# ElementsProject/lightning

Measured on NVIDIA H100. Metric: secp256k1 verifies/sec, higher is better.
Workload: dtype u32 (8x32-bit limbs, IMAD.WIDE.U32 carry chains)

## Files before the change

include/cln_sigverify.h:

```cpp
#ifndef CLN_SIGVERIFY_H
#define CLN_SIGVERIFY_H

#include <stddef.h>
#include <stdint.h>

#ifdef __cplusplus
extern "C" {
#endif

typedef struct sv_ctx sv_ctx;

#define SV_KIND_ECDSA33 0
#define SV_KIND_ECDSA_XY 1
#define SV_KIND_SCHNORR 2

typedef enum {
    SV_OK = 0,
    SV_ERR_NO_DEVICE = -1,
    SV_ERR_CUDA = -2,
    SV_ERR_NOMEM = -3,
    SV_ERR_ARG = -4,
    SV_ERR_IO = -5
} sv_status;

// ... 156 lines not shown
    uint64_t input_amount, output_amount;
    uint32_t prevouts_off, prevouts_len;
    uint32_t sequences_off, sequences_len;
} sv_tx;
int sv_verify_tx_host(sv_ctx *ctx, int kind, const sv_tx *txs, const uint8_t *scripts, size_t scripts_len,
                      const uint8_t *key, const uint8_t *sig64, size_t n, uint8_t *verdicts, uint8_t *sighash32_out);

int sv_grind_tx_fee_host(sv_ctx *ctx, int kind, const sv_tx *tx, const uint8_t *scripts, size_t scripts_len,
                         const uint8_t *key, const uint8_t *sig64, uint64_t weight, uint32_t min_feerate,
                         uint32_t max_feerate, int64_t *feerate_out, uint64_t *fee_out);

int sv_verify_bolt12_host(sv_ctx *ctx, const char *messagename, const char *fieldname, const uint8_t *blob,
                          size_t blob_len, const uint64_t *off, const uint32_t *len, const uint8_t *xonly32,
                          const uint8_t *sig64, size_t n, int *status, uint8_t *sighash32_out);
int sv_verify_bolt12_tagged_host(sv_ctx *ctx, size_t ntags, const char *const *messagenames, const char *const *fieldnames,
                                 const uint32_t *tag_of, const uint8_t *blob, size_t blob_len, const uint64_t *off,
                                 const uint32_t *len, const uint8_t *xonly32, const uint8_t *sig64, size_t n,
                                 int *status, uint8_t *sighash32_out);

int sv_verify_bolt11_host(sv_ctx *ctx, const uint8_t *blob, size_t blob_len, const uint64_t *off, const uint32_t *len,
                          size_t n, int *status, uint8_t *node_id33_out, uint8_t *hash32_out);

int sv_verify_device(sv_ctx *ctx, int kind, const void *d_msg32, const void *d_key, const void *d_sig64, size_t n,
                     void *d_verdicts, void *d_bitmap, void *stream);
int sv_sync(sv_ctx *ctx, void *stream);
void *sv_get_stream(const sv_ctx *ctx);

long sv_enqueue(sv_ctx *ctx, int kind, const uint8_t msg32[32], const uint8_t *key, const uint8_t sig64[64]);
size_t sv_pending(const sv_ctx *ctx);
int sv_flush(sv_ctx *ctx, uint8_t *verdicts, size_t capacity);

int sv_sha256d_host(sv_ctx *ctx, const uint8_t *data, size_t data_len, const uint64_t *off, const uint32_t *len,
                    size_t n, uint8_t *out32);
int sv_pubkey_parse_host(sv_ctx *ctx, const uint8_t *key33, size_t n, uint8_t *xy64, uint8_t *ok);

enum {
    SV_ST_FE_MUL = 0,
    SV_ST_FE_SQR = 1,
    SV_ST_FE_ADD = 2,
    SV_ST_FE_SUB = 3,
    SV_ST_FE_NEG = 4,
    SV_ST_FE_NORMALIZE = 5,
    SV_ST_FE_INV = 6,
    SV_ST_FE_SQRT = 7,
    SV_ST_FE_MUL3 = 8,
    SV_ST_FE_MUL8 = 9,
    SV_ST_FE_MUL_SMALL = 10,
    SV_ST_FE_DBL = 11,
    SV_ST_FE_B32 = 12,
    SV_ST_U256_MUL_WIDE = 13,
    SV_ST_U256_SQR_WIDE = 14,
    SV_ST_FE_REDUCE512 = 15,
    SV_ST_U256_ADD = 16,
    SV_ST_U256_SUB = 17,
    SV_ST_SC_MUL = 20,
    SV_ST_SC_SQR = 21,
    SV_ST_SC_ADD = 22,
    SV_ST_SC_NEGATE = 23,
    SV_ST_SC_INVERSE = 24,
    SV_ST_SC_REDUCE512 = 25,
    SV_ST_SC_SPLIT_LAMBDA = 26,
    SV_ST_SC_SET_B32 = 27,
    SV_ST_ECMULT_GEN = 28,
    SV_ST_PREPARE_U2 = 29,
    SV_ST_PREPARE_U1 = 30,
    SV_ST_SC_INVERSE_VAR = 31,
    SV_ST_FE_INV_VAR = 32
};
int sv_selftest_host(sv_ctx *ctx, int op, const uint32_t *a, const uint32_t *b, size_t n, uint32_t *out);

#define SV_STG_IN_WORDS 64
#define SV_STG_OUT_WORDS 200
enum {
    SV_STG_GEJ_DOUBLE = 0,
    SV_STG_GEJ_ADD_GE = 1,
    SV_STG_GEJ_ADD_GEJ = 2,
    SV_STG_GE_SET_XO = 3,
    SV_STG_QTABLE_BUILD = 4,
    SV_STG_ECMULT_LADDER_Q = 5,
    SV_STG_ECMULT_HALF_LADDER = 6,
    SV_STG_ECMULT_COMB_ADD = 7,
    SV_STG_SMALL_COMB = 8,
    SV_STG_ECMULT_LADDER = 9,
    SV_STG_NS_LINEAR_FORM = 10
};
int sv_selftest_group_host(sv_ctx *ctx, int op, const uint32_t *in, size_t n, uint32_t *out);

int sv_synth_device(sv_ctx *ctx, int kind, uint64_t seed, size_t n, void *d_msg32, void *d_key, void *d_sig64,
                    void *stream);

typedef struct {
    int device;
    int sm_count;
    int main_block;
    int main_grid;
    int main_regs;
    size_t gtable_bytes;
    size_t scratch_bytes;
    unsigned long long launches;
    size_t l2_persist_bytes;
    size_t l2_max_persist_bytes;
} sv_info;
int sv_get_info(const sv_ctx *ctx, sv_info *info);

int sv_set_profiling(sv_ctx *ctx, int on);
int sv_get_last_timing(sv_ctx *ctx, float *prep_ms, float *main_ms);
int sv_get_last_bolt12_timing(sv_ctx *ctx, float *merkle_ms, float *verify_ms);
int sv_get_last_bolt11_timing(sv_ctx *ctx, float *parse_ms, float *curve_ms);

int sv_probe_imad_peak(sv_ctx *ctx, double *imad_per_sec);
int sv_probe(sv_ctx *ctx, int mode, double *ops_per_sec);

void *sv_host_alloc(size_t bytes);
void sv_host_free(void *p);

#ifdef __cplusplus
}
#endif
#endif
```

lightning_b200/csrc/engine.cu:

```cuda
#include <cuda_runtime.h>
#include <cub/device/device_radix_sort.cuh>
#include <cub/device/device_scan.cuh>
#include <stdio.h>
#include <chrono>
#include <memory>
#include <stdlib.h>
#include <string.h>
#include <string>
#include <vector>

#include "../../include/cln_sigverify.h"
#include "verify.cuh"
#include "bolt12.cuh"
#include "bolt11.cuh"
#include "gossip_store.cuh"
#include "gossip_salvage.cuh"
#include "gossip_funding.cuh"
#include "selftest.cuh"
#include "batch.cuh"

#if !defined(SV_NO_SYNC_INLINE) && !defined(SV_FE_INLINE)
#error "compile with -DSV_FE_INLINE -DSV_MAIN_SYNC (default build) or -DSV_NO_SYNC_INLINE; see lightning_b200/build.py"
#endif
#ifdef SV_MAIN_SYNC
// ... 2980 lines not shown
    if (groups_total) *groups_total = groups;
    if (groups_failed) *groups_failed = failed;
    if (!idx.empty()) {
        size_t c = idx.size();
        CK(cudaMemcpyAsync(d_idx, idx.data(), 4 * c, cudaMemcpyHostToDevice, st));
        u8* g_msg = reinterpret_cast<u8*>(d_pts);
        u8* g_key = g_msg + 32 * c;
        u8* g_sig = g_key + 32 * c;
        u8* g_v = g_sig + 64 * c;
        k_sb_gather<<<(unsigned)((c + 255) / 256), 256, 0, st>>>(d_idx, c, ctx->d_msg, ctx->d_key, ctx->d_sig, g_msg, g_key, g_sig);
        ctx->launches += 1;
        rc = launch_verify(ctx, SV_KIND_SCHNORR, g_msg, g_key, g_sig, c, g_v, nullptr, st);
        if (rc) return rc;
        k_mixed_scatter<<<(unsigned)((c + 255) / 256), 256, 0, st>>>(d_idx, c, g_v, d_out);
        ctx->launches += 1;
        CK(cudaGetLastError());
    }
    CK(cudaMemcpyAsync(verdicts, d_out, n, cudaMemcpyDeviceToHost, st));
    CK(cudaStreamSynchronize(st));
    return SV_OK;
}

extern "C" long sv_enqueue(sv_ctx* ctx, int kind, const uint8_t msg32[32], const uint8_t* key, const uint8_t sig64[64]) {
    size_t ks = sv_key_size(kind);
    if (!ctx || ks == 0 || !msg32 || !key || !sig64) return SV_ERR_ARG;
    sv_queue_item it;
    it.kind = kind;
    memcpy(it.msg, msg32, 32);
    memset(it.key, 0, 64);
    memcpy(it.key, key, ks);
    memcpy(it.sig, sig64, 64);
    ctx->queue.push_back(it);
    return (long)ctx->queue.size() - 1;
}
extern "C" size_t sv_pending(const sv_ctx* ctx) { return ctx ? ctx->queue.size() : 0; }

extern "C" int sv_flush(sv_ctx* ctx, uint8_t* verdicts, size_t capacity) {
    if (!ctx || (!verdicts && !ctx->queue.empty())) return SV_ERR_ARG;
    size_t total = ctx->queue.size();
    if (capacity < total) return SV_ERR_ARG;
    for (int kind = 0; kind < 3; kind++) {
        size_t ks = sv_key_size(kind);
        std::vector<size_t> idx;
        for (size_t i = 0; i < total; i++)
            if (ctx->queue[i].kind == kind) idx.push_back(i);
        if (idx.empty()) continue;
        size_t m = idx.size();
        std::vector<u8> msg(32 * m), key(ks * m), sig(64 * m), out(m);
        for (size_t j = 0; j < m; j++) {
            const sv_queue_item& it = ctx->queue[idx[j]];
            memcpy(&msg[32 * j], it.msg, 32);
            memcpy(&key[ks * j], it.key, ks);
            memcpy(&sig[64 * j], it.sig, 64);
        }
        int rc = sv_verify_host(ctx, kind, msg.data(), key.data(), sig.data(), m, out.data());
        if (rc) return rc;
        for (size_t j = 0; j < m; j++) verdicts[idx[j]] = out[j];
    }
    ctx->queue.clear();
    return SV_OK;
}

extern "C" int sv_selftest_host(sv_ctx* ctx, int op, const uint32_t* a, const uint32_t* b, size_t n, uint32_t* out) {
    if (!ctx || op < 0 || op > SV_ST_FE_INV_VAR || (n && (!a || !b || !out))) return SV_ERR_ARG;
    if (n == 0) return SV_OK;
    dev_guard dg__;
    CK(dg__.enter(ctx->device));
    dev_buf<u32> ta, tb, to;
    int rc = ta.reserve(ctx, n * 32, n * 32);
    if (!rc) rc = tb.reserve(ctx, n * 32, n * 32);
    if (!rc) rc = to.reserve(ctx, n * 64, n * 64);
    if (rc) return rc;
    cudaStream_t st = ctx->stream;
    CK(cudaMemcpyAsync(ta, a, n * 32, cudaMemcpyHostToDevice, st));
    CK(cudaMemcpyAsync(tb, b, n * 32, cudaMemcpyHostToDevice, st));
    k_selftest<<<(unsigned)((n + 127) / 128), 128, 0, st>>>(op, ta, tb, n, to, ctx->d_gtab);
    ctx->launches += 1;
    CK(cudaGetLastError());
    CK(cudaMemcpyAsync(out, to, n * 64, cudaMemcpyDeviceToHost, st));
    CK(cudaStreamSynchronize(st));
    return SV_OK;
}
extern "C" int sv_selftest_group_host(sv_ctx* ctx, int op, const uint32_t* in, size_t n, uint32_t* out) {
    if (!ctx || op < 0 || op > SV_STG_NS_LINEAR_FORM || (n && (!in || !out))) return SV_ERR_ARG;
    if (n == 0) return SV_OK;
    dev_guard dg__;
    CK(dg__.enter(ctx->device));
    const size_t ib = n * 4 * SV_STG_IN_WORDS, ob = n * 4 * SV_STG_OUT_WORDS;
    dev_buf<u32> ti, to;
    int rc = ti.reserve(ctx, ib, ib);
    if (!rc) rc = to.reserve(ctx, ob, ob);
    if (rc) return rc;
    cudaStream_t st = ctx->stream;
    CK(cudaMemcpyAsync(ti, in, ib, cudaMemcpyHostToDevice, st));
    k_selftest_group<<<(unsigned)((n + 127) / 128), 128, 0, st>>>(op, ti, n, to, ctx->d_gtab);
    ctx->launches += 1;
    CK(cudaGetLastError());
    CK(cudaMemcpyAsync(out, to, ob, cudaMemcpyDeviceToHost, st));
    CK(cudaStreamSynchronize(st));
    return SV_OK;
}

extern "C" int sv_synth_device(sv_ctx* ctx, int kind, uint64_t seed, size_t n, void* d_msg32, void* d_key,
                               void* d_sig64, void* stream) {
    if (!ctx || sv_key_size(kind) == 0 || (n && (!d_msg32 || !d_key || !d_sig64))) return SV_ERR_ARG;
    if (n == 0) return SV_OK;
    dev_guard dg__;
    CK(dg__.enter(ctx->device));
    cudaStream_t st = stream ? (cudaStream_t)stream : ctx->stream;
    unsigned grid = (unsigned)((n + 127) / 128);
    if (kind == SV_KIND_ECDSA33)
        k_synth<SV_KIND_ECDSA33><<<grid, 128, 0, st>>>(seed, n, ctx->d_gtab, (u8*)d_msg32, (u8*)d_key, (u8*)d_sig64);
    else if (kind == SV_KIND_ECDSA_XY)
        k_synth<SV_KIND_ECDSA_XY><<<grid, 128, 0, st>>>(seed, n, ctx->d_gtab, (u8*)d_msg32, (u8*)d_key, (u8*)d_sig64);
    else
        k_synth<SV_KIND_SCHNORR><<<grid, 128, 0, st>>>(seed, n, ctx->d_gtab, (u8*)d_msg32, (u8*)d_key, (u8*)d_sig64);
    ctx->launches += 1;
    CK(cudaGetLastError());
    return SV_OK;
}

extern "C" int sv_probe(sv_ctx* ctx, int mode, double* ops_per_sec) {
    if (!ctx || !ops_per_sec || mode < 0 || mode > 10) return SV_ERR_ARG;
    dev_guard dg__;
    CK(dg__.enter(ctx->device));
    const int iters = (mode == 2 || mode == 3 || mode >= 9) ? 2000 : 4000;
    const int blocks = mode >= 9 ? 1 : ctx->sm_count * 8, threads = mode >= 9 ? 32 : 256;
    using event_ptr = std::unique_ptr<CUevent_st, cudaError_t (*)(cudaEvent_t)>;
    cudaEvent_t e0 = nullptr, e1 = nullptr;
    CK(cudaEventCreate(&e0));
    event_ptr own0(e0, cudaEventDestroy);
    CK(cudaEventCreate(&e1));
    event_ptr own1(e1, cudaEventDestroy);
    float best = 1e30f;
    for (int rep = 0; rep < 4; rep++) {
        CK(cudaEventRecord(e0, ctx->stream));
        switch (mode) {
            case 0: k_probe_imad_wide<<<blocks, threads, 0, ctx->stream>>>(iters, ctx->d_sink); break;
            case 1: k_probe_cmad4<<<blocks, threads, 0, ctx->stream>>>(iters, ctx->d_sink); break;
            case 2: k_probe_fe<0><<<blocks, threads, 0, ctx->stream>>>(iters, ctx->d_sink); break;
            case 3: k_probe_fe<1><<<blocks, threads, 0, ctx->stream>>>(iters, ctx->d_sink); break;
            case 4: k_probe_chain8<<<blocks, threads, 0, ctx->stream>>>(iters, ctx->d_sink); break;
            case 5: k_probe_carry_save<<<blocks, threads, 0, ctx->stream>>>(iters, ctx->d_sink); break;
            case 6: k_probe_imad32<<<blocks, threads, 0, ctx->stream>>>(iters, ctx->d_sink); break;
            case 8: k_probe_dfma<<<blocks, threads, 0, ctx->stream>>>(iters, ctx->d_sink); break;
            case 9: k_probe_fe<0><<<blocks, threads, 0, ctx->stream>>>(iters, ctx->d_sink); break;
            case 10: k_probe_fe<1><<<blocks, threads, 0, ctx->stream>>>(iters, ctx->d_sink); break;
            default: k_probe_addc<<<blocks, threads, 0, ctx->stream>>>(iters, ctx->d_sink); break;
        }
        CK(cudaEventRecord(e1, ctx->stream));
        CK(cudaEventSynchronize(e1));
        float ms = 0;
        CK(cudaEventElapsedTime(&ms, e0, e1));
        if (rep > 0 && ms < best) best = ms;
        ctx->launches += 1;
    }
    static const double per_iter[11] = {32.0, 32.0, 2.0, 2.0, 32.0, 32.0, 32.0, 64.0, 32.0, 2.0, 1.0};
    *ops_per_sec = per_iter[mode] * iters * (mode >= 9 ? 1.0 : (double)blocks * threads) / (best * 1e-3);
    return SV_OK;
}
extern "C" int sv_probe_imad_peak(sv_ctx* ctx, double* imad_per_sec) { return sv_probe(ctx, 0, imad_per_sec); }

extern "C" void* sv_host_alloc(size_t bytes) {
    void* p = nullptr;
    if (cudaHostAlloc(&p, bytes ? bytes : 1, cudaHostAllocDefault) != cudaSuccess) return nullptr;
    return p;
}
// ... 4 lines not shown
```

lightning_b200/csrc/fe.cuh:

```cuda
#pragma once
#include "u256.cuh"

struct fe {
    u32 v[8];
};

#define SV_P0 0xFFFFFC2Fu
#define SV_P1 0xFFFFFFFEu
#define SV_PC 977u

SV_HD void fe_set_zero(fe& r) {
    SV_UNROLL
    for (int i = 0; i < 8; i++) r.v[i] = 0;
}
SV_HD void fe_set_u32(fe& r, u32 x) {
    fe_set_zero(r);
    r.v[0] = x;
}

SV_HD bool fe_gte_p(const fe& a) {
    u32 hi = a.v[7] & a.v[6] & a.v[5] & a.v[4] & a.v[3] & a.v[2];
    return (hi == 0xFFFFFFFFu) && ((a.v[1] == 0xFFFFFFFFu) || (a.v[1] == SV_P1 && a.v[0] >= SV_P0));
}

// ... 31 lines not shown
    asm("mad.lo.cc.u32 %0, %3, 977, %0;\n\t"
        "addc.cc.u32 %1, %1, %3;\n\t"
        "addc.u32 %2, 0, 0;"
        : "+r"(r.v[0]), "+r"(r.v[1]), "=r"(k)
        : "r"(c));
    if (k) {
        u32 c2;
        asm("add.cc.u32 %0, %0, 1;\n\t"
            "addc.cc.u32 %1, %1, 0;\n\t"
            "addc.cc.u32 %2, %2, 0;\n\t"
            "addc.cc.u32 %3, %3, 0;\n\t"
            "addc.cc.u32 %4, %4, 0;\n\t"
            "addc.cc.u32 %5, %5, 0;\n\t"
            "addc.u32 %6, 0, 0;"
            : "+r"(r.v[2]), "+r"(r.v[3]), "+r"(r.v[4]), "+r"(r.v[5]), "+r"(r.v[6]), "+r"(r.v[7]), "=r"(c2));
        asm("mad.lo.cc.u32 %0, %2, 977, %0;\n\t"
            "addc.u32 %1, %1, %2;"
            : "+r"(r.v[0]), "+r"(r.v[1])
            : "r"(c2));
    }
#else
    u64 t = (u64)r.v[0] + (u64)c * SV_PC;
    r.v[0] = (u32)t;
    t = (u64)r.v[1] + c + (t >> 32);
    r.v[1] = (u32)t;
    for (int i = 2; i < 8; i++) { t = (u64)r.v[i] + (t >> 32); r.v[i] = (u32)t; }
    u32 c2 = (u32)(t >> 32);
    t = (u64)r.v[0] + (u64)c2 * SV_PC;
    r.v[0] = (u32)t;
    r.v[1] = (u32)((u64)r.v[1] + c2 + (t >> 32));
#endif
}

SV_HD void fe_sub(fe& r, const fe& a, const fe& b) {
    u32 bw = u256_sub(r.v, a.v, b.v);
#if SV_DEVICE_CODE
    u32 k;
    u32 kc = bw * SV_PC;
    asm("sub.cc.u32 %0, %0, %4;\n\t"
        "subc.cc.u32 %1, %1, %3;\n\t"
        "subc.u32 %2, 0, 0;"
        : "+r"(r.v[0]), "+r"(r.v[1]), "=r"(k)
        : "r"(bw), "r"(kc));
    if (k) {
        u32 b2;
        asm("sub.cc.u32 %0, %0, 1;\n\t"
            "subc.cc.u32 %1, %1, 0;\n\t"
            "subc.cc.u32 %2, %2, 0;\n\t"
            "subc.cc.u32 %3, %3, 0;\n\t"
            "subc.cc.u32 %4, %4, 0;\n\t"
            "subc.cc.u32 %5, %5, 0;\n\t"
            "subc.u32 %6, 0, 0;"
            : "+r"(r.v[2]), "+r"(r.v[3]), "+r"(r.v[4]), "+r"(r.v[5]), "+r"(r.v[6]), "+r"(r.v[7]), "=r"(b2));
        b2 &= 1u;
        u32 k2 = b2 * SV_PC;
        asm("sub.cc.u32 %0, %0, %3;\n\t"
            "subc.u32 %1, %1, %2;"
            : "+r"(r.v[0]), "+r"(r.v[1])
            : "r"(b2), "r"(k2));
    }
#else
    u64 d = (u64)r.v[0] - (u64)bw * SV_PC;
    r.v[0] = (u32)d;
    u64 br = (d >> 32) & 1;
    d = (u64)r.v[1] - bw - br;
    r.v[1] = (u32)d;
    br = (d >> 32) & 1;
    for (int i = 2; i < 8; i++) { d = (u64)r.v[i] - br; r.v[i] = (u32)d; br = (d >> 32) & 1; }
    u32 b2 = (u32)br;
    d = (u64)r.v[0] - (u64)b2 * SV_PC;
    r.v[0] = (u32)d;
    br = (d >> 32) & 1;
    r.v[1] = (u32)((u64)r.v[1] - b2 - br);
#endif
}

SV_HD void fe_neg(fe& r, const fe& a) {
    fe z;
    fe_set_zero(z);
    fe_sub(r, z, a);
}
SV_HD void fe_dbl(fe& r, const fe& a) { fe_add(r, a, a); }

SV_HD void fe_reduce512(fe& r, const u32 t[16]) {
#if SV_DEVICE_CODE
    u32 s[10];
    s[0] = t[0];
    asm("add.cc.u32 %0, %9, %17;\n\t"
        "addc.cc.u32 %1, %10, %18;\n\t"
        "addc.cc.u32 %2, %11, %19;\n\t"
        "addc.cc.u32 %3, %12, %20;\n\t"
        "addc.cc.u32 %4, %13, %21;\n\t"
        "addc.cc.u32 %5, %14, %22;\n\t"
        "addc.cc.u32 %6, %15, %23;\n\t"
        "addc.cc.u32 %7, %16, 0;\n\t"
        "addc.u32 %8, 0, 0;"
        : "=r"(s[1]), "=r"(s[2]), "=r"(s[3]), "=r"(s[4]), "=r"(s[5]), "=r"(s[6]), "=r"(s[7]), "=r"(s[8]), "=r"(s[9])
        : "r"(t[8]), "r"(t[9]), "r"(t[10]), "r"(t[11]), "r"(t[12]), "r"(t[13]), "r"(t[14]), "r"(t[15]),
          "r"(t[1]), "r"(t[2]), "r"(t[3]), "r"(t[4]), "r"(t[5]), "r"(t[6]), "r"(t[7]));
#ifdef SV_REDUCE_NOACC
    u32 pe[8];
    asm("mul.lo.u32 %0, %8, %12;\n\t"
        "mul.hi.u32 %1, %8, %12;\n\t"
        "mul.lo.u32 %2, %9, %12;\n\t"
        "mul.hi.u32 %3, %9, %12;\n\t"
        "mul.lo.u32 %4, %10, %12;\n\t"
        "mul.hi.u32 %5, %10, %12;\n\t"
        "mul.lo.u32 %6, %11, %12;\n\t"
        "mul.hi.u32 %7, %11, %12;"
        : "=r"(pe[0]), "=r"(pe[1]), "=r"(pe[2]), "=r"(pe[3]), "=r"(pe[4]), "=r"(pe[5]), "=r"(pe[6]), "=r"(pe[7])
        : "r"(t[8]), "r"(t[10]), "r"(t[12]), "r"(t[14]), "r"(SV_PC));
    asm("add.cc.u32 %0, %0, %10;\n\t"
        "addc.cc.u32 %1, %1, %11;\n\t"
        "addc.cc.u32 %2, %2, %12;\n\t"
        "addc.cc.u32 %3, %3, %13;\n\t"
        "addc.cc.u32 %4, %4, %14;\n\t"
        "addc.cc.u32 %5, %5, %15;\n\t"
        "addc.cc.u32 %6, %6, %16;\n\t"
        "addc.cc.u32 %7, %7, %17;\n\t"
        "addc.cc.u32 %8, %8, 0;\n\t"
        "addc.u32 %9, %9, 0;"
        : "+r"(s[0]), "+r"(s[1]), "+r"(s[2]), "+r"(s[3]), "+r"(s[4]), "+r"(s[5]), "+r"(s[6]), "+r"(s[7]),
          "+r"(s[8]), "+r"(s[9])
        : "r"(pe[0]), "r"(pe[1]), "r"(pe[2]), "r"(pe[3]), "r"(pe[4]), "r"(pe[5]), "r"(pe[6]), "r"(pe[7]));
#else
    asm("mad.lo.cc.u32 %0, %10, %14, %0;\n\t"
        "madc.hi.cc.u32 %1, %10, %14, %1;\n\t"
        "madc.lo.cc.u32 %2, %11, %14, %2;\n\t"
        "madc.hi.cc.u32 %3, %11, %14, %3;\n\t"
        "madc.lo.cc.u32 %4, %12, %14, %4;\n\t"
        "madc.hi.cc.u32 %5, %12, %14, %5;\n\t"
        "madc.lo.cc.u32 %6, %13, %14, %6;\n\t"
        "madc.hi.cc.u32 %7, %13, %14, %7;\n\t"
        "addc.cc.u32 %8, %8, 0;\n\t"
        "addc.u32 %9, %9, 0;"
        : "+r"(s[0]), "+r"(s[1]), "+r"(s[2]), "+r"(s[3]), "+r"(s[4]), "+r"(s[5]), "+r"(s[6]), "+r"(s[7]),
          "+r"(s[8]), "+r"(s[9])
        : "r"(t[8]), "r"(t[10]), "r"(t[12]), "r"(t[14]), "r"(SV_PC));
#endif
    u32 o[8];
    asm("mul.lo.u32 %0, %8, %12;\n\t"
        "mul.hi.u32 %1, %8, %12;\n\t"
        "mul.lo.u32 %2, %9, %12;\n\t"
        "mul.hi.u32 %3, %9, %12;\n\t"
        "mul.lo.u32 %4, %10, %12;\n\t"
        "mul.hi.u32 %5, %10, %12;\n\t"
        "mul.lo.u32 %6, %11, %12;\n\t"
        "mul.hi.u32 %7, %11, %12;"
        : "=r"(o[0]), "=r"(o[1]), "=r"(o[2]), "=r"(o[3]), "=r"(o[4]), "=r"(o[5]), "=r"(o[6]), "=r"(o[7])
        : "r"(t[9]), "r"(t[11]), "r"(t[13]), "r"(t[15]), "r"(SV_PC));
    asm("add.cc.u32 %0, %0, %9;\n\t"
        "addc.cc.u32 %1, %1, %10;\n\t"
        "addc.cc.u32 %2, %2, %11;\n\t"
        "addc.cc.u32 %3, %3, %12;\n\t"
        "addc.cc.u32 %4, %4, %13;\n\t"
        "addc.cc.u32 %5, %5, %14;\n\t"
        "addc.cc.u32 %6, %6, %15;\n\t"
        "addc.cc.u32 %7, %7, %16;\n\t"
        "addc.u32 %8, %8, 0;"
        : "+r"(s[1]), "+r"(s[2]), "+r"(s[3]), "+r"(s[4]), "+r"(s[5]), "+r"(s[6]), "+r"(s[7]), "+r"(s[8]), "+r"(s[9])
        : "r"(o[0]), "r"(o[1]), "r"(o[2]), "r"(o[3]), "r"(o[4]), "r"(o[5]), "r"(o[6]), "r"(o[7]));
    u64 T = ((u64)s[9] << 32) | s[8];
    u64 m = T * SV_PC;
    u64 mid = (m >> 32) + T;
    u32 f0 = (u32)m, f1 = (u32)mid, f2 = (u32)(mid >> 32);
    u32 c;
    asm("add.cc.u32 %0, %9, %17;\n\t"
        "addc.cc.u32 %1, %10, %18;\n\t"
        "addc.cc.u32 %2, %11, %19;\n\t"
        "addc.cc.u32 %3, %12, 0;\n\t"
        "addc.cc.u32 %4, %13, 0;\n\t"
        "addc.cc.u32 %5, %14, 0;\n\t"
        "addc.cc.u32 %6, %15, 0;\n\t"
        "addc.cc.u32 %7, %16, 0;\n\t"
        "addc.u32 %8, 0, 0;"
        : "=r"(r.v[0]), "=r"(r.v[1]), "=r"(r.v[2]), "=r"(r.v[3]), "=r"(r.v[4]), "=r"(r.v[5]), "=r"(r.v[6]),
          "=r"(r.v[7]), "=r"(c)
        : "r"(s[0]), "r"(s[1]), "r"(s[2]), "r"(s[3]), "r"(s[4]), "r"(s[5]), "r"(s[6]), "r"(s[7]), "r"(f0), "r"(f1),
          "r"(f2));
    asm("mad.lo.cc.u32 %0, %3, 977, %0;\n\t"
        "addc.cc.u32 %1, %1, %3;\n\t"
        "addc.u32 %2, %2, 0;"
        : "+r"(r.v[0]), "+r"(r.v[1]), "+r"(r.v[2])
        : "r"(c));
#else
    u64 acc = 0;
    u32 s[10];
    for (int i = 0; i < 8; i++) {
        acc += (u64)t[i] + (u64)t[8 + i] * SV_PC;
        if (i > 0) acc += t[8 + i - 1];
        s[i] = (u32)acc;
        acc >>= 32;
    }
    acc += t[15];
    s[8] = (u32)acc;
    s[9] = (u32)(acc >> 32);
    u64 T = ((u64)s[9] << 32) | s[8];
    u64 m = T * SV_PC;
    u64 mid = (m >> 32) + T;
    u32 f[3] = {(u32)m, (u32)mid, (u32)(mid >> 32)};
    u64 c = 0;
    for (int i = 0; i < 8; i++) {
        c += (u64)s[i] + (i < 3 ? f[i] : 0);
        r.v[i] = (u32)c;
        c >>= 32;
    }
    u32 cc = (u32)c;
    u64 q = (u64)r.v[0] + (u64)cc * SV_PC;
    r.v[0] = (u32)q;
    q = (u64)r.v[1] + cc + (q >> 32);
    r.v[1] = (u32)q;
    r.v[2] = (u32)((u64)r.v[2] + (q >> 32));
#endif
}

#if SV_DEVICE_CODE && !defined(SV_FE_INLINE)
static __device__ __noinline__ fe fe_mul_fn(fe a, fe b) {
    u32 t[16];
    fe r;
    u256_mul_wide(t, a.v, b.v);
    fe_reduce512(r, t);
    return r;
}
static __device__ __noinline__ fe fe_sqr_fn(fe a) {
    u32 t[16];
    fe r;
    u256_sqr_wide(t, a.v);
    fe_reduce512(r, t);
    return r;
}
SV_HD void fe_mul(fe& r, const fe& a, const fe& b) { r = fe_mul_fn(a, b); }
SV_HD void fe_sqr(fe& r, const fe& a) { r = fe_sqr_fn(a); }
#else
SV_HD void fe_mul(fe& r, const fe& a, const fe& b) {
    u32 t[16];
    u256_mul_wide(t, a.v, b.v);
    fe_reduce512(r, t);
}
SV_HD void fe_sqr(fe& r, const fe& a) {
    u32 t[16];
    u256_sqr_wide(t, a.v);
    fe_reduce512(r, t);
}
#endif

SV_HD void fe_mul_small(fe& r, const fe& a, u32 k) {
    u64 c = 0;
    u32 s[8];
    SV_UNROLL
    for (int i = 0; i < 8; i++) {
        c += (u64)a.v[i] * k;
        s[i] = (u32)c;
        c >>= 32;
    }
    u64 m = c * SV_PC;
    u64 q = (u64)s[0] + (u32)m;
    r.v[0] = (u32)q;
    q = (u64)s[1] + (m >> 32) + c + (q >> 32);
    r.v[1] = (u32)q;
    SV_UNROLL
    for (int i = 2; i < 8; i++) {
        q = (u64)s[i] + (q >> 32);
        r.v[i] = (u32)q;
    }
    u32 c2 = (u32)(q >> 32);
    q = (u64)r.v[0] + (u64)c2 * SV_PC;
    r.v[0] = (u32)q;
    q = (u64)r.v[1] + c2 + (q >> 32);
    r.v[1] = (u32)q;
    r.v[2] = (u32)((u64)r.v[2] + (q >> 32));
}

SV_HD void fe_mul3(fe& r, const fe& a) {
    fe t;
    fe_add(t, a, a);
    fe_add(r, t, a);
}
SV_HD void fe_mul8(fe& r, const fe& a) {
    u32 top = a.v[7] >> 29;
    u32 s[8];
    SV_UNROLL
    for (int i = 7; i > 0; i--) s[i] = (a.v[i] << 3) | (a.v[i - 1] >> 29);
    s[0] = a.v[0] << 3;
    u32 add0 = top * SV_PC;
    fe x, y;
    SV_UNROLL
    for (int i = 0; i < 8; i++) { x.v[i] = s[i]; y.v[i] = 0; }
    y.v[0] = add0;
    y.v[1] = top;
    fe_add(r, x, y);
}

SV_HD void fe_sqr_n(fe& r, const fe& a, int n) {
    r = a;
#if SV_DEVICE_CODE
// ... 89 lines not shown
```

lightning_b200/csrc/ge.cuh:

```cuda
#pragma once
#include "fe.cuh"

#define SV_GE_ADD_GENERIC 0
#define SV_GE_ADD_DOUBLE 1
#define SV_GE_ADD_INFINITY 2
#define SV_GE_ADD_A_INF 3
#define SV_GE_ADD_B_INF 4
#define SV_GE_MIXED 0
#define SV_GE_FULL 8
#ifndef SV_GE_TRACE
#define SV_GE_TRACE(ev) ((void)0)
#endif

struct ge {
    fe x, y;
};
struct gej {
    fe x, y, z;
    u32 inf;
};

static SV_CDATA const u32 GE_BETA[8] = {0x719501EEu, 0xC1396C28u, 0x12F58995u, 0x9CF04975u,
                                        0xAC3434E9u, 0x6E64479Eu, 0x657C0710u, 0x7AE96A2Bu};
static SV_CDATA const u32 GE_GX[8] = {0x16F81798u, 0x59F2815Bu, 0x2DCE28D9u, 0x029BFCDBu,
                                      0xCE870B07u, 0x55A06295u, 0xF9DCBBACu, 0x79BE667Eu};
static SV_CDATA const u32 GE_GY[8] = {0xFB10D4B8u, 0x9C47D08Fu, 0xA6855419u, 0xFD17B448u,
                                      0x0E1108A8u, 0x5DA4FBFCu, 0x26A3C465u, 0x483ADA77u};

SV_HD void gej_set_ge(gej& r, const ge& a) {
    r.x = a.x;
    r.y = a.y;
    fe_set_u32(r.z, 1);
    r.inf = 0;
}

SV_HD void gej_double(gej& r, const gej& a) {
    fe A, B, C, D, E, t;
    fe_sqr(A, a.x);
    fe_sqr(B, a.y);
    fe_sqr(C, B);
    fe_add(t, a.x, B);
    fe_sqr(t, t);
    fe_sub(t, t, A);
    fe_sub(t, t, C);
    fe_dbl(D, t);
    fe_mul3(E, A);
    fe_mul(t, a.y, a.z);
    fe_dbl(r.z, t);
    fe_sqr(t, E);
    fe_sub(t, t, D);
    fe_sub(r.x, t, D);
    fe_sub(t, D, r.x);
    fe_mul(t, t, E);
    fe_mul8(C, C);
    fe_sub(r.y, t, C);
    r.inf = a.inf;
}

SV_HD void gej_add_ge(gej& r, const gej& a, const ge& b, fe* rzr = nullptr) {
    if (a.inf) {
        SV_GE_TRACE(SV_GE_MIXED | SV_GE_ADD_A_INF);
        gej_set_ge(r, b);
        if (rzr) fe_set_u32(*rzr, 1);
        return;
    }
    fe zz, u2, s2, h, rr, hh, hhh, v, t;
    fe_sqr(zz, a.z);
    fe_mul(u2, b.x, zz);
    fe_mul(t, a.z, zz);
    fe_mul(s2, b.y, t);
    fe_sub(h, u2, a.x);
    fe_sub(rr, s2, a.y);
    if (fe_is_zero(h)) {
        if (fe_is_zero(rr)) {
            SV_GE_TRACE(SV_GE_MIXED | SV_GE_ADD_DOUBLE);
            if (rzr) fe_dbl(*rzr, a.y);
            gej_double(r, a);
        } else {
            SV_GE_TRACE(SV_GE_MIXED | SV_GE_ADD_INFINITY);
            r.inf = 1;
            if (rzr) fe_set_zero(*rzr);
        }
        return;
    }
    SV_GE_TRACE(SV_GE_MIXED | SV_GE_ADD_GENERIC);
    if (rzr) *rzr = h;
    fe_sqr(hh, h);
    fe_mul(hhh, h, hh);
    fe_mul(v, a.x, hh);
    fe_mul(r.z, a.z, h);
    fe_sqr(t, rr);
    fe_sub(t, t, hhh);
    fe_sub(t, t, v);
    fe x3;
    fe_sub(x3, t, v);
    fe_sub(t, v, x3);
    fe_mul(t, t, rr);
    fe_mul(hhh, hhh, a.y);
    fe_sub(r.y, t, hhh);
    r.x = x3;
    r.inf = 0;
}

SV_HD void gej_add_gej(gej& r, const gej& a, const gej& b) {
    if (a.inf) {
        SV_GE_TRACE(SV_GE_FULL | SV_GE_ADD_A_INF);
        r = b;
        return;
    }
    if (b.inf) {
        SV_GE_TRACE(SV_GE_FULL | SV_GE_ADD_B_INF);
        r = a;
        return;
    }
    fe z22, z12, u1, u2, s1, s2, h, rr, t;
    fe_sqr(z22, b.z);
    fe_sqr(z12, a.z);
    fe_mul(u1, a.x, z22);
    fe_mul(u2, b.x, z12);
    fe_mul(t, b.z, z22);
    fe_mul(s1, a.y, t);
    fe_mul(t, a.z, z12);
    fe_mul(s2, b.y, t);
    fe_sub(h, u2, u1);
    fe_sub(rr, s2, s1);
    if (fe_is_zero(h)) {
        if (fe_is_zero(rr)) {
            SV_GE_TRACE(SV_GE_FULL | SV_GE_ADD_DOUBLE);
            gej_double(r, a);
        } else {
            SV_GE_TRACE(SV_GE_FULL | SV_GE_ADD_INFINITY);
            r.inf = 1;
            fe_set_zero(r.x);
            fe_set_zero(r.y);
            fe_set_zero(r.z);
        }
        return;
    }
// ... 51 lines not shown
```

lightning_b200/csrc/selftest.cuh:

```cuda
#pragma once
#include "../../include/cln_sigverify.h"
#include "verify.cuh"

SV_HD void selftest_item(int op, const u32 A[8], const u32 B[8], u32 R[16], const ge_mem* gtab) {
    SV_UNROLL
    for (int k = 0; k < 16; k++) R[k] = 0;
    fe x, y, r;
    sc p, q, s;
SV_UNROLL
    for (int k = 0; k < 8; k++) { x.v[k] = A[k]; y.v[k] = B[k]; p.v[k] = A[k]; q.v[k] = B[k]; }
    fe_set_zero(r);
    bool is_fe = false, is_sc = false;
    switch (op) {
        case SV_ST_FE_MUL: fe_mul(r, x, y); is_fe = true; break;
        case SV_ST_FE_SQR: fe_sqr(r, x); is_fe = true; break;
        case SV_ST_FE_ADD: fe_add(r, x, y); is_fe = true; break;
        case SV_ST_FE_SUB: fe_sub(r, x, y); is_fe = true; break;
        case SV_ST_FE_NEG: fe_neg(r, x); is_fe = true; break;
        case SV_ST_FE_NORMALIZE: r = x; fe_normalize(r); is_fe = true; R[8] = fe_is_zero(x); R[9] = fe_gte_p(x); R[10] = fe_equal(x, y); break;
        case SV_ST_FE_INV: fe_inv(r, x); is_fe = true; break;
        case SV_ST_FE_SQRT: R[8] = fe_sqrt(r, x) ? 1u : 0u; is_fe = true; break;
        case SV_ST_FE_MUL3: fe_mul3(r, x); is_fe = true; break;
        case SV_ST_FE_MUL8: fe_mul8(r, x); is_fe = true; break;
        case SV_ST_FE_MUL_SMALL: fe_mul_small(r, x, B[0] & 0xFFFFu); is_fe = true; break;
// ... 122 lines not shown
            break;
        case SV_STG_GEJ_ADD_GE: {
            fe rzr;
            fe_set_zero(rzr);
            stg_load_gej(a, in);
            stg_load_fe(q.x, in + 32);
            stg_load_fe(q.y, in + 40);
            r = a;
            if (in[60] & 1u) gej_add_ge(r, r, q, &rzr); else gej_add_ge(r, a, q, &rzr);
            stg_store_gej(out, r);
            stg_store_fe(out + 32, rzr);
            break;
        }
        case SV_STG_GEJ_ADD_GEJ:
            stg_load_gej(a, in);
            stg_load_gej(b, in + 32);
            if (in[60] == 1u) { gej_add_gej(a, a, b); r = a; }
            else if (in[60] == 2u) { gej_add_gej(b, a, b); r = b; }
            else gej_add_gej(r, a, b);
            stg_store_gej(out, r);
            break;
        case SV_STG_GE_SET_XO: {
            fe x;
            stg_load_fe(x, in);
            out[16] = ge_set_xo(q, x, in[8] != 0) ? 1u : 0u;
            stg_store_fe(out, q.x);
            stg_store_fe(out + 8, q.y);
            break;
        }
        case SV_STG_QTABLE_BUILD:
            stg_load_fe(q.x, in);
            stg_load_fe(q.y, in + 8);
            qtable_build(tab, zc, q);
            for (int e = 0; e < 8; e++)
                for (int k = 0; k < 8; k++) { out[24 * e + k] = tab[e].x[k]; out[24 * e + 8 + k] = tab[e].y[k]; out[24 * e + 16 + k] = tab[e].h[k]; }
            stg_store_fe(out + 192, zc);
            break;
        case SV_STG_ECMULT_LADDER_Q:
        case SV_STG_ECMULT_HALF_LADDER:
        case SV_STG_ECMULT_LADDER: {
            sv_work w;
            stg_load_work(w, in);
            stg_load_fe(q.x, in);
            stg_load_fe(q.y, in + 8);
            qtable_build(tab, zc, q);
            if (op == SV_STG_ECMULT_LADDER_Q) ecmult_ladder_q(r, &w, tab, zc);
            else if (op == SV_STG_ECMULT_LADDER) ecmult_ladder(r, &w, gtab, tab, zc);
            else ecmult_half_ladder(r, w.k1, in[60] != 0, tab);
            stg_store_gej(out, r);
            stg_store_fe(out + 32, zc);
            break;
        }
        case SV_STG_ECMULT_COMB_ADD: {
            sv_work w;
            stg_load_work(w, in);
            stg_load_gej(r, in);
            ecmult_comb_add(r, &w, gtab);
            stg_store_gej(out, r);
            break;
        }
        case SV_STG_SMALL_COMB: {
            sv_small_item it;
            stg_load_work(it.w, in);
            small_comb(&it, gtab);
            small_jac_load(r, &it.p3);
            stg_store_gej(out, r);
            break;
        }
        case SV_STG_NS_LINEAR_FORM: {
            fe X1, Y1, Zs, c, rfe, D, B, ext[2];
            stg_load_fe(X1, in);
            stg_load_fe(Y1, in + 8);
            stg_load_fe(Zs, in + 16);
            stg_load_fe(c, in + 24);
            stg_load_gej(b, in + 32);
            stg_load_fe(rfe, in + 56);
            out[32] = ns_linear_form(D, B, X1, Y1, Zs, b, c, rfe, ext) ? 1u : 0u;
            stg_store_fe(out, D);
            stg_store_fe(out + 8, B);
            stg_store_fe(out + 16, ext[0]);
            stg_store_fe(out + 24, ext[1]);
            break;
        }
        default: break;
    }
}
```

lightning_b200/csrc/verify.cuh:

```cuda
#pragma once
#include "ge.cuh"
#include "sc.cuh"
#include "sha256.cuh"

#define SV_KIND_ECDSA33 0
#define SV_KIND_ECDSA_XY 1
#define SV_KIND_SCHNORR 2
#define SV_KIND_ECDSA33_NS 3
#define SV_KIND_SCHNORR_NS 4

#define SV_GT_ROW 32768
#define SV_GT_ENTRIES (15 * SV_GT_ROW + 65536)

struct alignas(16) ge_mem {
    u32 x[8], y[8];
};
struct alignas(16) qtab_entry {
    u32 x[8], y[8], h[8];
};

SV_HD void ge_from_mem(ge& r, const ge_mem* p) {
#if SV_DEVICE_CODE
    const uint4* q = reinterpret_cast<const uint4*>(p);
    uint4 a = q[0], b = q[1], c = q[2], d = q[3];
// ... 152 lines not shown
    fe_sqr(c2, D.z);
    fe_mul(c3, c2, D.z);
    ge d_aff, q1;
    d_aff.x = D.x;
    d_aff.y = D.y;
    fe_mul(q1.x, Q.x, c2);
    fe_mul(q1.y, Q.y, c3);
    gej_set_ge(acc, q1);
    fe_to_words(tab[0].x, q1.x);
    fe_to_words(tab[0].y, q1.y);
#if SV_DEVICE_CODE
#pragma unroll 1
#endif
    for (int k = 1; k < 8; k++) {
        fe h;
        SV_SYNC(sync_threads);
        gej_add_ge(acc, acc, d_aff, &h);
        fe_to_words(tab[k].x, acc.x);
        fe_to_words(tab[k].y, acc.y);
        fe_to_words(tab[k].h, h);
    }
    fe_mul(zc, acc.z, D.z);
    fe zr;
    fe_from_words(zr, tab[7].h);
#if SV_DEVICE_CODE
#pragma unroll 1
#endif
    for (int k = 6; k >= 0; k--) {
        fe zr2, zr3, t;
        fe_sqr(zr2, zr);
        fe_mul(zr3, zr2, zr);
        fe_from_words(t, tab[k].x);
        fe_mul(t, t, zr2);
        fe_to_words(tab[k].x, t);
        fe_from_words(t, tab[k].y);
        fe_mul(t, t, zr3);
        fe_to_words(tab[k].y, t);
        if (k > 0) {
            fe_from_words(t, tab[k].h);
            fe_mul(zr, zr, t);
        }
    }
    fe beta;
    SV_UNROLL
    for (int i = 0; i < 8; i++) beta.v[i] = GE_BETA[i];
#if SV_DEVICE_CODE
#pragma unroll 1
#endif
    for (int k = 0; k < 8; k++) {
        fe t;
        fe_from_words(t, tab[k].x);
        fe_mul(t, t, beta);
        fe_to_words(tab[k].h, t);
    }
}

SV_HD void qtable_fetch(ge& p, const qtab_entry* tab, u32 v, u32 sneg, bool lam) {
    u32 dneg = (v < 8) ? 1u : 0u;
    u32 idx = dneg ? (7u - v) : (v - 8u);
    fe_from_words(p.x, lam ? tab[idx].h : tab[idx].x);
    fe_from_words(p.y, tab[idx].y);
    if (dneg ^ sneg) fe_neg(p.y, p.y);
}

SV_HD void ecmult_ladder_q(gej& R, const sv_work* w, const qtab_entry* tab, const fe& zc, unsigned sync_threads = 0) {
    const u32* m1 = w->k1;
    const u32* m2 = w->k2;
    u32 t1 = m1[4], t2 = m2[4];
    u32 s1 = t1 >> 31, s2 = t2 >> 31;
    ge p;
    {
        u32 v1 = (t1 >> 1) & 7u, v2 = (t2 >> 1) & 7u;
        qtable_fetch(p, tab, v1 + 8u, s1, false);
        gej_set_ge(R, p);
        qtable_fetch(p, tab, v2 + 8u, s2, true);
        gej_add_ge(R, R, p);
    }
#if SV_DEVICE_CODE
#pragma unroll 1
#endif
    for (int i = 31; i >= 0; i--) {
        if (i % 2 == 0) SV_SYNC(sync_threads);
        for (int j = 0; j < 4; j++) {
            gej_double(R, R);
        }
#if SV_DEVICE_CODE
#pragma unroll 1
#endif
        for (int half = 0; half < 2; half++) {
            u32 v = half ? window4(m2, i) : window4(m1, i);
            qtable_fetch(p, tab, v, half ? s2 : s1, half != 0);
            gej_add_ge(R, R, p);
        }
    }
    fe_mul(R.z, R.z, zc);
}

SV_HD void ecmult_comb_add(gej& R, const sv_work* w, const ge_mem* gtab, unsigned sync_threads = 0) {
    ge p;
#if SV_DEVICE_CODE
#pragma unroll 1
#endif
    for (int row = 0; row < 16; row++) {
        int d = w->gd[row];
        SV_SYNC(sync_threads);
        if (d != 0) {
            u32 a = (u32)(d < 0 ? -d : d);
            ge_from_mem(p, gtab + (size_t)row * SV_GT_ROW + (a - 1));
            if (d < 0) fe_neg(p.y, p.y);
            gej_add_ge(R, R, p);
        }
    }
}

SV_HD void ecmult_ladder(gej& R, const sv_work* w, const ge_mem* gtab, const qtab_entry* tab, const fe& zc,
                         unsigned sync_threads = 0) {
    ecmult_ladder_q(R, w, tab, zc, sync_threads);
    ecmult_comb_add(R, w, gtab, sync_threads);
}

SV_HD void ecmult_uniform(gej& R, const sv_work* w, const ge& Q, const ge_mem* gtab, qtab_entry* tab,
                          unsigned sync_threads = 0) {
    fe zc;
    qtable_build(tab, zc, Q, sync_threads);
    ecmult_ladder(R, w, gtab, tab, zc, sync_threads);
}

SV_HD u32 ecdsa_final(const gej& R, const u8* sig64, u32 flags);

struct alignas(16) sv_shared_key {
    qtab_entry tab[8];
    u32 zc[8];
    u32 ok, pad[3];
};
SV_HD void sharedkey_build(sv_shared_key* out, int kind, const u8* key, unsigned sync_threads = 0) {
    ge Q;
    bool ok = key_decode(Q, kind, key);
    fe zc;
    qtable_build(out->tab, zc, Q, sync_threads);
    fe_to_words(out->zc, zc);
    out->ok = ok ? 1u : 0u;
}
SV_HD u32 verify_curve_side_shared(const sv_work* w, const u8* sig64, const ge_mem* gtab, const sv_shared_key* sk,
                                   unsigned sync_threads = 0) {
    u32 flags = w->flags;
    bool ok = (flags & SV_WF_VALID) != 0 && sk->ok != 0;
    fe zc;
    fe_from_words(zc, sk->zc);
    gej R;
    ecmult_ladder(R, w, gtab, sk->tab, zc, sync_threads);
    u32 v = ecdsa_final(R, sig64, flags);
    return ok ? v : 0u;
}

SV_HD u32 ecdsa_final(const gej& R, const u8* sig64, u32 flags) {
    if (R.inf) return 0;
    fe xr, zz, t;
    fe_set_b32(xr, sig64);
    fe_sqr(zz, R.z);
    fe_mul(t, xr, zz);
    if (fe_equal(t, R.x)) return 1;
    if (flags & SV_WF_R_PLUS_N) {
        fe nn;
        SV_UNROLL
        for (int i = 0; i < 8; i++) nn.v[i] = SC_N[i];
        u256_add(xr.v, xr.v, nn.v);
        fe_mul(t, xr, zz);
// ... 889 lines not shown
```

Baseline: 46.29 million.

## Use lazy-reduction point doubling in ecmult ladder with wide subtract-then-reduce

Adds a gej_double_ladder that keeps intermediate products unreduced at 512-bit width, subtracting a shifted wide C=B^2 before a single reduction, fusing reductions in the S and Y3 computations. A generalized fe_reduce_wide handles the extra top limb, and the non-accumulating reduce path becomes unconditional instead of the mad-chain variant. The ladder's doublings now use this routine, aiming to cut reductions per doubling at the cost of more register pressure from 16-limb temporaries. Selftest ops are added to check the new routines.

```diff
diff --git a/include/cln_sigverify.h b/include/cln_sigverify.h
--- a/include/cln_sigverify.h
+++ b/include/cln_sigverify.h
@@ -262,7 +262,9 @@
     SV_STG_ECMULT_COMB_ADD = 7,
     SV_STG_SMALL_COMB = 8,
     SV_STG_ECMULT_LADDER = 9,
-    SV_STG_NS_LINEAR_FORM = 10
+    SV_STG_NS_LINEAR_FORM = 10,
+    SV_STG_FE_WIDE = 11,
+    SV_STG_GEJ_DOUBLE_LADDER = 12
 };
 int sv_selftest_group_host(sv_ctx *ctx, int op, const uint32_t *in, size_t n, uint32_t *out);
 
diff --git a/lightning_b200/csrc/engine.cu b/lightning_b200/csrc/engine.cu
--- a/lightning_b200/csrc/engine.cu
+++ b/lightning_b200/csrc/engine.cu
@@ -3086,7 +3086,7 @@
     return SV_OK;
 }
 extern "C" int sv_selftest_group_host(sv_ctx* ctx, int op, const uint32_t* in, size_t n, uint32_t* out) {
-    if (!ctx || op < 0 || op > SV_STG_NS_LINEAR_FORM || (n && (!in || !out))) return SV_ERR_ARG;
+    if (!ctx || op < 0 || op > SV_STG_GEJ_DOUBLE_LADDER || (n && (!in || !out))) return SV_ERR_ARG;
     if (n == 0) return SV_OK;
     dev_guard dg__;
     CK(dg__.enter(ctx->device));
diff --git a/lightning_b200/csrc/fe.cuh b/lightning_b200/csrc/fe.cuh
--- a/lightning_b200/csrc/fe.cuh
+++ b/lightning_b200/csrc/fe.cuh
@@ -137,7 +137,7 @@
 }
 SV_HD void fe_dbl(fe& r, const fe& a) { fe_add(r, a, a); }
 
-SV_HD void fe_reduce512(fe& r, const u32 t[16]) {
+SV_HD void fe_reduce_wide(fe& r, const u32 t[16], u32 top) {
 #if SV_DEVICE_CODE
     u32 s[10];
     s[0] = t[0];
@@ -153,7 +153,6 @@
         : "=r"(s[1]), "=r"(s[2]), "=r"(s[3]), "=r"(s[4]), "=r"(s[5]), "=r"(s[6]), "=r"(s[7]), "=r"(s[8]), "=r"(s[9])
         : "r"(t[8]), "r"(t[9]), "r"(t[10]), "r"(t[11]), "r"(t[12]), "r"(t[13]), "r"(t[14]), "r"(t[15]),
           "r"(t[1]), "r"(t[2]), "r"(t[3]), "r"(t[4]), "r"(t[5]), "r"(t[6]), "r"(t[7]));
-#ifdef SV_REDUCE_NOACC
     u32 pe[8];
     asm("mul.lo.u32 %0, %8, %12;\n\t"
         "mul.hi.u32 %1, %8, %12;\n\t"
@@ -178,21 +177,6 @@
         : "+r"(s[0]), "+r"(s[1]), "+r"(s[2]), "+r"(s[3]), "+r"(s[4]), "+r"(s[5]), "+r"(s[6]), "+r"(s[7]),
           "+r"(s[8]), "+r"(s[9])
         : "r"(pe[0]), "r"(pe[1]), "r"(pe[2]), "r"(pe[3]), "r"(pe[4]), "r"(pe[5]), "r"(pe[6]), "r"(pe[7]));
-#else
-    asm("mad.lo.cc.u32 %0, %10, %14, %0;\n\t"
-        "madc.hi.cc.u32 %1, %10, %14, %1;\n\t"
-        "madc.lo.cc.u32 %2, %11, %14, %2;\n\t"
-        "madc.hi.cc.u32 %3, %11, %14, %3;\n\t"
-        "madc.lo.cc.u32 %4, %12, %14, %4;\n\t"
-        "madc.hi.cc.u32 %5, %12, %14, %5;\n\t"
-        "madc.lo.cc.u32 %6, %13, %14, %6;\n\t"
-        "madc.hi.cc.u32 %7, %13, %14, %7;\n\t"
-        "addc.cc.u32 %8, %8, 0;\n\t"
-        "addc.u32 %9, %9, 0;"
-        : "+r"(s[0]), "+r"(s[1]), "+r"(s[2]), "+r"(s[3]), "+r"(s[4]), "+r"(s[5]), "+r"(s[6]), "+r"(s[7]),
-          "+r"(s[8]), "+r"(s[9])
-        : "r"(t[8]), "r"(t[10]), "r"(t[12]), "r"(t[14]), "r"(SV_PC));
-#endif
     u32 o[8];
     asm("mul.lo.u32 %0, %8, %12;\n\t"
         "mul.hi.u32 %1, %8, %12;\n\t"
@@ -215,7 +199,7 @@
         "addc.u32 %8, %8, 0;"
         : "+r"(s[1]), "+r"(s[2]), "+r"(s[3]), "+r"(s[4]), "+r"(s[5]), "+r"(s[6]), "+r"(s[7]), "+r"(s[8]), "+r"(s[9])
         : "r"(o[0]), "r"(o[1]), "r"(o[2]), "r"(o[3]), "r"(o[4]), "r"(o[5]), "r"(o[6]), "r"(o[7]));
-    u64 T = ((u64)s[9] << 32) | s[8];
+    u64 T = (((u64)s[9] << 32) | s[8]) + (((u64)top << 32) | (top * SV_PC));
     u64 m = T * SV_PC;
     u64 mid = (m >> 32) + T;
     u32 f0 = (u32)m, f1 = (u32)mid, f2 = (u32)(mid >> 32);
@@ -250,7 +234,7 @@
     acc += t[15];
     s[8] = (u32)acc;
     s[9] = (u32)(acc >> 32);
-    u64 T = ((u64)s[9] << 32) | s[8];
+    u64 T = (((u64)s[9] << 32) | s[8]) + (((u64)top << 32) | (top * SV_PC));
     u64 m = T * SV_PC;
     u64 mid = (m >> 32) + T;
     u32 f[3] = {(u32)m, (u32)mid, (u32)(mid >> 32)};
@@ -266,6 +250,77 @@
     q = (u64)r.v[1] + cc + (q >> 32);
     r.v[1] = (u32)q;
     r.v[2] = (u32)((u64)r.v[2] + (q >> 32));
+#endif
+}
+
+SV_HD void fe_reduce512(fe& r, const u32 t[16]) { fe_reduce_wide(r, t, 0); }
+
+template <int S>
+SV_HD u32 fe_wide_sub(u32 r[16], const u32 a[16], const u32 c[16]) {
+    static_assert(S >= 0 && S <= 3, "shift");
+    const u32 P8[8] = {SV_P0, SV_P1, 0xFFFFFFFFu, 0xFFFFFFFFu, 0xFFFFFFFFu, 0xFFFFFFFFu, 0xFFFFFFFFu, 0xFFFFFFFFu};
+    u32 k[9], cs[17];
+    k[0] = P8[0] << (S + 1);
+    SV_UNROLL
+    for (int i = 1; i < 8; i++) k[i] = (P8[i] << (S + 1)) | (P8[i - 1] >> (31 - S));
+    k[8] = P8[7] >> (31 - S);
+    if constexpr (S == 0) {
+        SV_UNROLL
+        for (int i = 0; i < 16; i++) cs[i] = c[i];
+        cs[16] = 0;
+    } else {
+        cs[0] = c[0] << S;
+        SV_UNROLL
+        for (int i = 1; i < 16; i++) cs[i] = (c[i] << S) | (c[i - 1] >> (32 - S));
+        cs[16] = c[15] >> (32 - S);
+    }
+#if SV_DEVICE_CODE
+    u32 h[9], top;
+    asm("add.cc.u32 %0, %9, %17;\n\t"
+        "addc.cc.u32 %1, %10, %18;\n\t"
+        "addc.cc.u32 %2, %11, %19;\n\t"
+        "addc.cc.u32 %3, %12, %20;\n\t"
+        "addc.cc.u32 %4, %13, %21;\n\t"
+        "addc.cc.u32 %5, %14, %22;\n\t"
+        "addc.cc.u32 %6, %15, %23;\n\t"
+        "addc.cc.u32 %7, %16, %24;\n\t"
+        "addc.u32 %8, %25, 0;"
+        : "=r"(h[0]), "=r"(h[1]), "=r"(h[2]), "=r"(h[3]), "=r"(h[4]), "=r"(h[5]), "=r"(h[6]), "=r"(h[7]), "=r"(h[8])
+        : "r"(a[8]), "r"(a[9]), "r"(a[10]), "r"(a[11]), "r"(a[12]), "r"(a[13]), "r"(a[14]), "r"(a[15]),
+          "r"(k[0]), "r"(k[1]), "r"(k[2]), "r"(k[3]), "r"(k[4]), "r"(k[5]), "r"(k[6]), "r"(k[7]), "r"(k[8]));
+    asm("sub.cc.u32 %0, %17, %34;\n\t"
+        "subc.cc.u32 %1, %18, %35;\n\t"
+        "subc.cc.u32 %2, %19, %36;\n\t"
+        "subc.cc.u32 %3, %20, %37;\n\t"
+        "subc.cc.u32 %4, %21, %38;\n\t"
+        "subc.cc.u32 %5, %22, %39;\n\t"
+        "subc.cc.u32 %6, %23, %40;\n\t"
+        "subc.cc.u32 %7, %24, %41;\n\t"
+        "subc.cc.u32 %8, %25, %42;\n\t"
+        "subc.cc.u32 %9, %26, %43;\n\t"
+        "subc.cc.u32 %10, %27, %44;\n\t"
+        "subc.cc.u32 %11, %28, %45;\n\t"
+        "subc.cc.u32 %12, %29, %46;\n\t"
+        "subc.cc.u32 %13, %30, %47;\n\t"
+        "subc.cc.u32 %14, %31, %48;\n\t"
+        "subc.cc.u32 %15, %32, %49;\n\t"
+        "subc.u32 %16, %33, %50;"
+        : "=r"(r[0]), "=r"(r[1]), "=r"(r[2]), "=r"(r[3]), "=r"(r[4]), "=r"(r[5]), "=r"(r[6]), "=r"(r[7]), "=r"(r[8]),
+          "=r"(r[9]), "=r"(r[10]), "=r"(r[11]), "=r"(r[12]), "=r"(r[13]), "=r"(r[14]), "=r"(r[15]), "=r"(top)
+        : "r"(a[0]), "r"(a[1]), "r"(a[2]), "r"(a[3]), "r"(a[4]), "r"(a[5]), "r"(a[6]), "r"(a[7]), "r"(h[0]), "r"(h[1]),
+          "r"(h[2]), "r"(h[3]), "r"(h[4]), "r"(h[5]), "r"(h[6]), "r"(h[7]), "r"(h[8]), "r"(cs[0]), "r"(cs[1]), "r"(cs[2]),
+          "r"(cs[3]), "r"(cs[4]), "r"(cs[5]), "r"(cs[6]), "r"(cs[7]), "r"(cs[8]), "r"(cs[9]), "r"(cs[10]), "r"(cs[11]),
+          "r"(cs[12]), "r"(cs[13]), "r"(cs[14]), "r"(cs[15]), "r"(cs[16]));
+    return top;
+#else
+    int64_t acc = 0;
+    for (int i = 0; i < 17; i++) {
+        acc += (int64_t)(i < 16 ? a[i] : 0u) + (int64_t)(i >= 8 ? k[i - 8] : 0u) - (int64_t)cs[i];
+        if (i < 16) r[i] = (u32)acc;
+        else return (u32)acc;
+        acc >>= 32;
+    }
+    return 0;
 #endif
 }
 
diff --git a/lightning_b200/csrc/ge.cuh b/lightning_b200/csrc/ge.cuh
--- a/lightning_b200/csrc/ge.cuh
+++ b/lightning_b200/csrc/ge.cuh
@@ -54,6 +54,32 @@
     fe_mul(t, t, E);
     fe_mul8(C, C);
     fe_sub(r.y, t, C);
+    r.inf = a.inf;
+}
+
+SV_HD void gej_double_ladder(gej& r, const gej& a) {
+    fe A, B, D, E, t, x3, y3, z3;
+    u32 C[16], w[16];
+    fe_sqr(A, a.x);
+    fe_sqr(B, a.y);
+    u256_sqr_wide(C, B.v);
+    fe_add(t, a.x, B);
+    u256_sqr_wide(w, t.v);
+    fe_reduce_wide(t, w, fe_wide_sub<0>(w, w, C));
+    fe_sub(t, t, A);
+    fe_dbl(D, t);
+    fe_mul3(E, A);
+    fe_mul(t, a.y, a.z);
+    fe_dbl(z3, t);
+    fe_sqr(t, E);
+    fe_sub(t, t, D);
+    fe_sub(x3, t, D);
+    fe_sub(t, D, x3);
+    u256_mul_wide(w, t.v, E.v);
+    fe_reduce_wide(y3, w, fe_wide_sub<3>(w, w, C));
+    r.x = x3;
+    r.y = y3;
+    r.z = z3;
     r.inf = a.inf;
 }
 
diff --git a/lightning_b200/csrc/selftest.cuh b/lightning_b200/csrc/selftest.cuh
--- a/lightning_b200/csrc/selftest.cuh
+++ b/lightning_b200/csrc/selftest.cuh
@@ -228,6 +228,31 @@
             stg_store_fe(out + 24, ext[1]);
             break;
         }
+        case SV_STG_FE_WIDE: {
+            fe x, y, u, v;
+            u32 t[16], w[16], d[16];
+            stg_load_fe(x, in);
+            stg_load_fe(y, in + 8);
+            stg_load_fe(u, in + 16);
+            stg_load_fe(v, in + 24);
+            for (int k = 0; k < 16; k++) t[k] = in[32 + k];
+            fe_reduce_wide(zc, t, in[48]);
+            stg_store_fe(out, zc);
+            u256_mul_wide(t, x.v, y.v);
+            u256_mul_wide(w, u.v, v.v);
+            fe_reduce_wide(zc, d, fe_wide_sub<0>(d, t, w));
+            stg_store_fe(out + 8, zc);
+            fe_reduce_wide(zc, d, fe_wide_sub<1>(d, t, w));
+            stg_store_fe(out + 16, zc);
+            fe_reduce_wide(zc, d, fe_wide_sub<3>(d, t, w));
+            stg_store_fe(out + 24, zc);
+            break;
+        }
+        case SV_STG_GEJ_DOUBLE_LADDER:
+            stg_load_gej(a, in);
+            gej_double_ladder(r, a);
+            stg_store_gej(out, r);
+            break;
         default: break;
     }
 }
diff --git a/lightning_b200/csrc/verify.cuh b/lightning_b200/csrc/verify.cuh
--- a/lightning_b200/csrc/verify.cuh
+++ b/lightning_b200/csrc/verify.cuh
@@ -258,7 +258,7 @@
     for (int i = 31; i >= 0; i--) {
         if (i % 2 == 0) SV_SYNC(sync_threads);
         for (int j = 0; j < 4; j++) {
-            gej_double(R, R);
+            gej_double_ladder(R, R);
         }
 #if SV_DEVICE_CODE
 #pragma unroll 1
```

Measured after the change: 47.23 million (median of 6 runs). +2.0%, better.
